# RolandFaure/metagenome_vector_sketches

Measured on AMD Instinct MI355X. Metric: samples projected/sec + pairwise Jaccard cells/sec, d=2048, 1/2/4/8 GPUs, higher is better.
Workload: dtype u64 hash -> int32 sketch; int8 limbs x int32 MFMA accumulate; fp64 keep test

## Files before the change

### metagenome_vector_sketches_amd/csrc/mvs_capi.hip

```cpp
#include "mvs_capi_internal.h"

using namespace mvs_capi;

namespace mvs {
int capi_fail(int code, const char* fmt, ...);
hipStream_t capi_stream(mvs_ctx* c) { return c->stream; }
int capi_device(mvs_ctx* c) { return c->device; }
const Options& capi_options(mvs_ctx* c) { return c->opt; }
}

namespace {
thread_local std::string g_err;
}

std::atomic<unsigned long long> mvs_capi::g_set_ids{0};

int mvs_capi::fail(int code, const char* fmt, ...) {
    char buf[512];
    va_list ap;
    va_start(ap, fmt);
    vsnprintf(buf, sizeof buf, fmt, ap);
    va_end(ap);
    g_err = buf;
    return code;
}

int mvs::capi_fail(int code, const char* fmt, ...) {
    char buf[512];
    va_list ap;
    va_start(ap, fmt);
    vsnprintf(buf, sizeof buf, fmt, ap);
    va_end(ap);
    g_err = buf;
    return code;
}

namespace {

struct Roctx {
    int (*push)(const char*) = nullptr;
    int (*pop)() = nullptr;
    Roctx() {
        for (const char* name : {"librocprofiler-sdk-roctx.so.1", "librocprofiler-sdk-roctx.so", "libroctx64.so.4",
                                 "libroctx64.so", "/opt/rocm/lib/librocprofiler-sdk-roctx.so"}) {
            if (void* h = dlopen(name, RTLD_NOW | RTLD_LOCAL)) {
                push = reinterpret_cast<int (*)(const char*)>(dlsym(h, "roctxRangePushA"));
                pop = reinterpret_cast<int (*)()>(dlsym(h, "roctxRangePop"));
                if (push && pop) return;
                push = nullptr;
                pop = nullptr;
            }
        }
    }
};
const Roctx& roctx() {
    static const Roctx r;
    return r;
}

}

namespace mvs_capi {

Range::Range(const mvs_ctx* c, const char* name) {
    if (c && c->opt.markers && roctx().push) {
        roctx().push(name);
        on = true;
    }
}
Range::~Range() {
    if (on) roctx().pop();
}

int ensure_buf(mvs_ctx* c, void** p, size_t* have, size_t bytes) {
    if (*have >= bytes) return MVS_OK;
    if (*p) {
        HIP_TRY(hipStreamSynchronize(c->stream));
        HIP_TRY(hipFree(*p));
        *p = nullptr;
        *have = 0;
    }
    const size_t want = bytes + std::min<size_t>(bytes / 4, (size_t)256 << 20) + 4096;
    if (hipMalloc(p, want) != hipSuccess) return fail(MVS_E_NOMEM, "hipMalloc of %zu bytes failed", want);
    *have = want;
    return MVS_OK;
}

int ensure_read_back(mvs_ctx* c, size_t total) {
    if (c->rb_pinned && c->rb_bytes >= total) return MVS_OK;
    if (c->rb_pinned) HIP_TRY(hipHostFree(c->rb_pinned));
    c->rb_pinned = nullptr;
    c->rb_bytes = 0;
    const size_t want = std::max<size_t>(total * 2, (size_t)1 << 20);
    HIP_TRY(hipHostMalloc(&c->rb_pinned, want, hipHostMallocDefault));
    c->rb_bytes = want;
    return MVS_OK;
}
int read_back(mvs_ctx* c, hipStream_t st, std::initializer_list<ReadBack> items) {
    size_t total = 0;
    for (const ReadBack& it : items) total += (it.bytes + 63) & ~(size_t)63;
    const int rc_rb = ensure_read_back(c, total);
    if (rc_rb) return rc_rb;
    size_t at = 0;
    for (const ReadBack& it : items) {
        if (it.bytes) HIP_TRY(hipMemcpyAsync((char*)c->rb_pinned + at, it.src, it.bytes, hipMemcpyDeviceToHost, st));
        at += (it.bytes + 63) & ~(size_t)63;
    }
    HIP_TRY(hipStreamSynchronize(st));
    at = 0;
    for (const ReadBack& it : items) {
        if (it.bytes) memcpy(it.dst, (const char*)c->rb_pinned + at, it.bytes);
        at += (it.bytes + 63) & ~(size_t)63;
    }
    return MVS_OK;
}

int ensure_scratch(mvs_ctx* c, size_t bytes) {
    if (c->scratch_bytes >= bytes) return MVS_OK;
    if (c->scratch) {
        HIP_TRY(hipStreamSynchronize(c->stream));
        HIP_TRY(hipFree(c->scratch));
        c->scratch = nullptr;
        c->scratch_bytes = 0;
    }
    HIP_TRY(hipMalloc(&c->scratch, bytes));
    c->scratch_bytes = bytes;
    return MVS_OK;
}

int acquire_pinned(mvs_ctx* c, size_t bytes) {
    if (c->pinned_busy) {
        HIP_TRY(hipEventSynchronize(c->pinned_ev));
        c->pinned_busy = false;
    }
    if (c->pinned_bytes >= bytes) return MVS_OK;
    if (c->pinned) {
        HIP_TRY(hipHostFree(c->pinned));
        c->pinned = nullptr;
        c->pinned_bytes = 0;
    }
    const size_t want = bytes < (1u << 20) ? (1u << 20) : bytes;
    HIP_TRY(hipHostMalloc(&c->pinned, want, hipHostMallocDefault));
    c->pinned_bytes = want;
    return MVS_OK;
}

struct OptionSpec {
    const char* name;
    int mvs::Options::*ifield;
    double mvs::Options::*dfield;
    long long lo, hi;
};
const OptionSpec kOptions[] = {
    {"pairwise_filter", &mvs::Options::pairwise_filter, nullptr, 0, 2},
    {"filter_variant", &mvs::Options::filter_variant, nullptr, -1, 99},
    {"exact_variant", &mvs::Options::exact_variant, nullptr, 0, 3},
    {"pairwise_variant", &mvs::Options::pairwise_variant, nullptr, 0, 9},
    {"pairwise_symmetric", &mvs::Options::pairwise_symmetric, nullptr, 0, 1},
    {"pairwise_debug", &mvs::Options::pairwise_debug, nullptr, 0, 15},
    {"sort", &mvs::Options::sort, nullptr, 0, 2},
    {"enable_k3", &mvs::Options::enable_k3, nullptr, 0, 1},
    {"markers", &mvs::Options::markers, nullptr, 0, 1},
    {"project_variant", &mvs::Options::project_variant, nullptr, 0, 14},
    {"comm_timeout_s", &mvs::Options::comm_timeout_s, nullptr, 1, 86400},
    {"pairwise_map", &mvs::Options::pairwise_map, nullptr, 0, 2},
    {"coarse_radix", &mvs::Options::coarse_radix, nullptr, 0, 1},
    {"cand_regions", &mvs::Options::cand_regions, nullptr, 0, 1},
    {"recheck_mode", &mvs::Options::recheck_mode, nullptr, 0, 3},
    {"recheck_blocks", &mvs::Options::recheck_blocks, nullptr, 1, 64},
    {"stream_dense", &mvs::Options::stream_dense, nullptr, 0, 5},
    {"encode_stage_words", &mvs::Options::encode_stage_words, nullptr, 1, 64},
    {"stream_block_rows", &mvs::Options::stream_block_rows, nullptr, 0, 1 << 30},
    {"tile_dense_thr", &mvs::Options::tile_dense_thr, nullptr, 0, 8192},
    {"stream_list_cells", &mvs::Options::stream_list_cells, nullptr, 0, 1 << 30},
    {"stream_pipeline", &mvs::Options::stream_pipeline, nullptr, 0, 1},
    {"stream_trace", &mvs::Options::stream_trace, nullptr, 0, 1},
    {"search_stream", &mvs::Options::search_stream, nullptr, 0, 1},
    {"search_depth", &mvs::Options::search_depth, nullptr, 3, 6},
    {"fragment_major", &mvs::Options::fragment_major, nullptr, 0, 1},
    {"pairwise_bdirect", &mvs::Options::pairwise_bdirect, nullptr, 0, 1},
    {"plan_strip_wgs", &mvs::Options::plan_strip_wgs, nullptr, 256, 1 << 22},
    {"recode_rows_wg", &mvs::Options::recode_rows_wg, nullptr, 8, 16},
    {"plan_speculate", &mvs::Options::plan_speculate, nullptr, 0, 1},
    {"plan_order", &mvs::Options::plan_order, nullptr, 0, 1},
    {"stream_piece_mib", &mvs::Options::stream_piece_mib, nullptr, 1, 1024},
    {"stream_spec", &mvs::Options::stream_spec, nullptr, 0, 1},
    {"stream_copy", &mvs::Options::stream_copy, nullptr, 0, 1},
    {"topk_dots", &mvs::Options::topk_dots, nullptr, 0, 1},
    {"topk_block_rows", &mvs::Options::topk_block_rows, nullptr, 0, 1 << 30},
    {"pairwise_block_cells", nullptr, &mvs::Options::pairwise_block_cells, 1, (1LL << 62)},
};

int apply_option(mvs::Options& o, const OptionSpec& sp, long long v) {
#ifndef MVS_ABLATIONS
    if (sp.ifield == &mvs::Options::pairwise_debug && v != 0)
        return fail(MVS_E_INVALID, "pairwise_debug needs a library built with -DMVS_ABLATIONS");
    if (sp.ifield == &mvs::Options::filter_variant && v >= 11 && v <= 33)
        return fail(MVS_E_INVALID, "filter_variant %lld is a k-loop ablation: needs -DMVS_ABLATIONS", v);
#endif
    if (v < sp.lo || v > sp.hi) return fail(MVS_E_INVALID, "option %s: %lld outside [%lld, %lld]", sp.name, v, sp.lo, sp.hi);
    if (sp.ifield) o.*(sp.ifield) = (int)v;
    else o.*(sp.dfield) = (double)v;
    return MVS_OK;
}

void options_from_env(mvs::Options& o) {
    for (const OptionSpec& sp : kOptions) {
        std::string env = "MVS_";
        for (const char* p = sp.name; *p; ++p) env += (char)toupper((unsigned char)*p);
        const char* e = getenv(env.c_str());
        if (!e || !*e) continue;
        long long v;
        if (sp.ifield == &mvs::Options::sort && (e[0] == 'm' || e[0] == 'r')) v = e[0] == 'r' ? 2 : 1;
        else v = sp.dfield ? (long long)atof(e) : atoll(e);
        const std::string keep = g_err;
        if (apply_option(o, sp, v) != MVS_OK) g_err = keep;
    }
}

void parallel_copy(void* dst, const void* src, size_t bytes) {
    const size_t kMin = 8u << 20;
    unsigned nt = std::thread::hardware_concurrency();
    nt = nt == 0 ? 4 : (nt > 16 ? 16 : nt);
    if (bytes < 2 * kMin) nt = 1;
    if (nt <= 1) {
        std::memcpy(dst, src, bytes);
        return;
    }
    std::vector<std::thread> pool;
    const size_t per = (bytes / nt + 4095) & ~(size_t)4095;
    for (unsigned t = 0; t < nt; ++t) {
        const size_t b = (size_t)t * per;
        if (b >= bytes) break;
        const size_t n = std::min(per, bytes - b);
        pool.emplace_back([=]() { std::memcpy((char*)dst + b, (const char*)src + b, n); });
    }
    for (auto& th : pool) th.join();
}

int ensure_upload_pipeline(mvs_ctx* c) {
    if (c->up_bytes) return MVS_OK;
    HIP_TRY(hipStreamCreateWithFlags(&c->up_stream, hipStreamNonBlocking));
    for (int i = 0; i < 2; ++i) {
        HIP_TRY(hipHostMalloc(&c->up_pinned[i], kUploadPiece, hipHostMallocDefault));
        HIP_TRY(hipEventCreateWithFlags(&c->up_done[i], hipEventDisableTiming));
    }
    c->up_bytes = kUploadPiece;
    return MVS_OK;
}

int check_kernel(const char* what) {
    hipError_t e = hipGetLastError();
    if (e != hipSuccess) return fail(MVS_E_HIP, "%s launch: %s", what, hipGetErrorString(e));
    return MVS_OK;
}

}

extern "C" {

const char* mvs_version(void) { return "mvs_hip 0.1 (gfx950)"; }
const char* mvs_last_error(void) { return g_err.c_str(); }

int mvs_device_count(int* count) {
    if (!count) return fail(MVS_E_INVALID, "count is NULL");
    int n = 0;
    hipError_t e = hipGetDeviceCount(&n);
    if (e != hipSuccess) {
        *count = 0;
        return fail(MVS_E_HIP, "hipGetDeviceCount: %s", hipGetErrorString(e));
    }
    *count = n;
    return MVS_OK;
}

int mvs_ctx_create(int device, mvs_ctx** out) {
    if (!out) return fail(MVS_E_INVALID, "ctx out pointer is NULL");
    *out = nullptr;
    int n = 0;
    hipError_t e = hipGetDeviceCount(&n);
    if (e != hipSuccess || n <= 0)
        return fail(MVS_E_HIP, "no HIP device available (%s); libmvs_hip has no CPU fallback",
                    e != hipSuccess ? hipGetErrorString(e) : "device count 0");
    if (device < 0 || device >= n) return fail(MVS_E_INVALID, "device %d out of range [0,%d)", device, n);
    HIP_TRY(hipSetDevice(device));
    hipDeviceProp_t prop;
    HIP_TRY(hipGetDeviceProperties(&prop, device));
    if (std::strncmp(prop.gcnArchName, "gfx950", 6) != 0)
        return fail(MVS_E_HIP, "device %d is %s; this library is built for gfx950 only", device, prop.gcnArchName);
    mvs_ctx* c = new (std::nothrow) mvs_ctx();
    if (!c) return fail(MVS_E_NOMEM, "out of host memory");
    c->device = device;
#ifdef MVS_ABLATIONS
    c->opt.pairwise_bdirect = 0;
#endif
    options_from_env(c->opt);
    if (hipStreamCreateWithFlags(&c->own_stream, hipStreamNonBlocking) != hipSuccess) {
        delete c;
        return fail(MVS_E_HIP, "hipStreamCreate failed");
    }
    c->stream = c->own_stream;
    for (auto& ev : c->ev) {
        if (hipEventCreate(&ev) != hipSuccess) {
            mvs_ctx_destroy(c);
            return fail(MVS_E_HIP, "hipEventCreate failed");
        }
    }
    if (hipEventCreateWithFlags(&c->pinned_ev, hipEventDisableTiming) != hipSuccess) {
        mvs_ctx_destroy(c);
        return fail(MVS_E_HIP, "hipEventCreate failed");
    }
    if (hipMalloc((void**)&c->d_counter, 2048) != hipSuccess) {
        mvs_ctx_destroy(c);
        return fail(MVS_E_HIP, "hipMalloc failed");
    }
    *out = c;
// ... 264 lines not shown
```

### metagenome_vector_sketches_amd/csrc/mvs_capi_sketch.hip

```cpp
#include "mvs_capi_internal.h"

using namespace mvs_capi;

extern "C" {

int mvs_project_csr(mvs_ctx* c, const uint64_t* hashes, int mem_hashes, const int64_t* offsets,
                    int64_t n_samples, int d, int32_t* out, int mem_out) {
    return mvs_project_csr_stats(c, hashes, mem_hashes, offsets, n_samples, d, out, mem_out, nullptr, nullptr);
}

int mvs_project_csr_stats(mvs_ctx* c, const uint64_t* hashes, int mem_hashes, const int64_t* offsets,
                          int64_t n_samples, int d, int32_t* out, int mem_out, int64_t* sumsq, int64_t* max_abs) {
    if (!c) return fail(MVS_E_INVALID, "ctx is NULL");
    const Range range(c, "mvs_project_csr");
    if ((sumsq == nullptr) != (max_abs == nullptr)) return fail(MVS_E_INVALID, "sumsq and max_abs go together");
    int64_t* const sumsq_user = sumsq;
    DevBuf dsum;
    if (max_abs) *max_abs = 0;
    if (n_samples < 0 || d <= 0) return fail(MVS_E_INVALID, "n_samples=%lld d=%d", (long long)n_samples, d);
    if (!mem_ok(mem_hashes) || !mem_ok(mem_out)) return fail(MVS_E_INVALID, "bad mem flag");
    if (n_samples == 0) return MVS_OK;
    if (!offsets || !out) return fail(MVS_E_INVALID, "offsets/out is NULL");
    HIP_TRY(hipSetDevice(c->device));

    if (n_samples >= (1LL << 31)) return fail(MVS_E_RANGE, "too many samples");
    size_t n_units = 0;
    bool all_single = true;
    for (int64_t s = 0; s < n_samples; ++s) {
        const int64_t b = offsets[s], e = offsets[s + 1];
        if (e < b) return fail(MVS_E_INVALID, "offsets not monotone at sample %lld", (long long)s);
        if (e - b >= (1LL << 31)) return fail(MVS_E_RANGE, "sample %lld has >= 2^31 hashes", (long long)s);
        n_units += e == b ? 1 : (size_t)((e - b + mvs::kProjUnitMax - 1) / mvs::kProjUnitMax);
        all_single = all_single && (e - b) <= mvs::kProjUnitMax;
    }
    int rc = acquire_pinned(c, std::max<size_t>(n_units * sizeof(mvs::ProjUnit), 256));
    if (rc) return rc;
    mvs::ProjUnit* units = (mvs::ProjUnit*)c->pinned;
    {
        size_t w = 0;
        for (int64_t s = 0; s < n_samples; ++s) {
            const int64_t b = offsets[s], e = offsets[s + 1];
            const bool single = (e - b) <= mvs::kProjUnitMax;
            if (e == b) units[w++] = mvs::ProjUnit{b, 0, (int32_t)s, 1, 0};
            for (int64_t p = b; p < e; p += mvs::kProjUnitMax) {
                mvs::ProjUnit u;
                u.begin = p;
                u.count = (int32_t)std::min<int64_t>(mvs::kProjUnitMax, e - p);
                u.sample = (int32_t)s;
                u.single = single ? 1 : 0;
                u.pad = 0;
                units[w++] = u;
            }
        }
    }
    const int64_t total = offsets[n_samples];
    if (total > 0 && !hashes) return fail(MVS_E_INVALID, "hashes is NULL");

    DevBuf dh, dout;
    const uint64_t* d_hashes = hashes;
    const bool pipelined = mem_hashes == MVS_MEM_HOST && (size_t)total * 8 > kUploadPiece;
    if (mem_hashes == MVS_MEM_HOST) {
        HIP_TRY(dh.alloc((size_t)total * 8));
        if (!pipelined) HIP_TRY(hipMemcpyAsync(dh.p, hashes, (size_t)total * 8, hipMemcpyHostToDevice, c->stream));
        d_hashes = (const uint64_t*)dh.p;
    }
    int32_t* d_out = out;
    const size_t out_bytes = (size_t)n_samples * (size_t)d * 4;
    if (mem_out == MVS_MEM_HOST) {
        HIP_TRY(dout.alloc(out_bytes));
        d_out = (int32_t*)dout.p;
        if (sumsq) {
            HIP_TRY(dsum.alloc((size_t)n_samples * 8));
            sumsq = (int64_t*)dsum.p;
        }
    }
    const size_t ubytes = n_units * sizeof(mvs::ProjUnit);
    rc = ensure_scratch(c, std::max<size_t>(ubytes, 256));
    if (rc) return rc;
    if (n_units) {
        HIP_TRY(hipMemcpyAsync(c->scratch, units, ubytes, hipMemcpyHostToDevice, c->stream));
        HIP_TRY(hipEventRecord(c->pinned_ev, c->stream));
        c->pinned_busy = true;
    }

    if (!all_single) HIP_TRY(hipMemsetAsync(d_out, 0, out_bytes, c->stream));
    const bool fused = sumsq != nullptr && all_single;
    if (fused) {
        HIP_TRY(hipMemsetAsync(sumsq, 0, (size_t)n_samples * 8, c->stream));
        HIP_TRY(hipMemsetAsync(c->d_counter, 0, 8, c->stream));
    }
    if (c->timing) HIP_TRY(hipEventRecord(c->ev[0], c->stream));
    const int nblk = (d + 63) / 64;
    int bpw = (nblk % 4 == 0 && nblk >= 8) ? 14 : (nblk >= 2 ? 2 : 1);
    if (c->opt.project_variant == 14 && nblk >= 4) bpw = 14;
    if (c->opt.project_variant == 12 && nblk >= 2) bpw = 12;
    if (c->opt.project_variant == 2 && nblk >= 2) bpw = 2;
    if (c->opt.project_variant == 1) bpw = 1;
    if (!pipelined) {
        mvs::launch_project(c->stream, d_hashes, (const mvs::ProjUnit*)c->scratch, (int64_t)n_units, d, d_out, bpw,
                            fused ? (unsigned long long*)sumsq : nullptr, fused ? c->d_counter : nullptr);
        rc = check_kernel("k_project");
        if (rc) return rc;
    } else {
        rc = ensure_upload_pipeline(c);
        if (rc) return rc;
        size_t u_done = 0;
        const size_t total_bytes = (size_t)total * 8;
        int piece = 0;
        for (size_t off = 0; off < total_bytes; off += kUploadPiece, ++piece) {
            const int b = piece & 1;
            const size_t len = std::min(kUploadPiece, total_bytes - off);
            if (piece >= 2) HIP_TRY(hipEventSynchronize(c->up_done[b]));
            parallel_copy(c->up_pinned[b], (const char*)hashes + off, len);
            HIP_TRY(hipMemcpyAsync((char*)dh.p + off, c->up_pinned[b], len, hipMemcpyHostToDevice, c->up_stream));
            HIP_TRY(hipEventRecord(c->up_done[b], c->up_stream));
            const int64_t covered = (int64_t)((off + len) / 8);
            size_t u_next = u_done;
            while (u_next < n_units && units[u_next].begin + units[u_next].count <= covered) ++u_next;
            if (u_next > u_done) {
                HIP_TRY(hipStreamWaitEvent(c->stream, c->up_done[b], 0));
                mvs::launch_project(c->stream, d_hashes, (const mvs::ProjUnit*)c->scratch + u_done, (int64_t)(u_next - u_done), d,
                                    d_out, bpw, fused ? (unsigned long long*)sumsq : nullptr, fused ? c->d_counter : nullptr);
                rc = check_kernel("k_project");
                if (rc) return rc;
                u_done = u_next;
            }
        }
        if (u_done != n_units) return fail(MVS_E_INVALID, "internal: %zu of %zu projection units launched", u_done, n_units);
    }
    if (c->timing) {
        HIP_TRY(hipEventRecord(c->ev[1], c->stream));
        c->ev_valid[0] = true;
    }
    if (sumsq) {
        if (fused) {
            unsigned long long m = 0;
            {
                const int rb_rc = read_back(c, c->stream, {{&m, c->d_counter, 8}});
                if (rb_rc) return rb_rc;
            }
            *max_abs = (int64_t)m;
        } else {
            rc = mvs_sketch_stats(c, d_out, MVS_MEM_DEVICE, n_samples, d, sumsq, MVS_MEM_DEVICE, max_abs);
            if (rc) return rc;
        }
    }
    if (mem_out == MVS_MEM_HOST) {
        HIP_TRY(hipMemcpyAsync(out, d_out, out_bytes, hipMemcpyDeviceToHost, c->stream));
        if (sumsq_user) HIP_TRY(hipMemcpyAsync(sumsq_user, sumsq, (size_t)n_samples * 8, hipMemcpyDeviceToHost, c->stream));
        HIP_TRY(hipStreamSynchronize(c->stream));
    } else if (mem_hashes == MVS_MEM_HOST) {
        HIP_TRY(hipStreamSynchronize(c->stream));
    } else {
    }
    return MVS_OK;
}

int mvs_sketch_sumsq(mvs_ctx* c, const int32_t* sketches, int mem_in, int64_t n, int d, int64_t* sumsq,
                     int mem_out) {
    if (!c) return fail(MVS_E_INVALID, "ctx is NULL");
    if (n < 0 || d <= 0 || !mem_ok(mem_in) || !mem_ok(mem_out)) return fail(MVS_E_INVALID, "bad argument");
    if (n == 0) return MVS_OK;
    if (!sketches || !sumsq) return fail(MVS_E_INVALID, "NULL buffer");
    HIP_TRY(hipSetDevice(c->device));
    DevBuf din, dout;
    const int32_t* d_in = sketches;
    if (mem_in == MVS_MEM_HOST) {
        HIP_TRY(din.alloc((size_t)n * d * 4));
        HIP_TRY(hipMemcpyAsync(din.p, sketches, (size_t)n * d * 4, hipMemcpyHostToDevice, c->stream));
        d_in = (const int32_t*)din.p;
    }
    int64_t* d_out = sumsq;
    if (mem_out == MVS_MEM_HOST) {
        HIP_TRY(dout.alloc((size_t)n * 8));
        d_out = (int64_t*)dout.p;
    }
    mvs::launch_sumsq(c->stream, d_in, n, d, d_out);
    int rc = check_kernel("k_sumsq");
    if (rc) return rc;
    if (mem_out == MVS_MEM_HOST)
        HIP_TRY(hipMemcpyAsync(sumsq, d_out, (size_t)n * 8, hipMemcpyDeviceToHost, c->stream));
    if (mem_out == MVS_MEM_HOST || mem_in == MVS_MEM_HOST) HIP_TRY(hipStreamSynchronize(c->stream));
    return MVS_OK;
}

}

namespace mvs_capi {

__device__ double norm_sq_from_text(long long sumsq, int d) {
    if (sumsq <= 0) return 0.0;
    const double x = sqrt((double)sumsq / (double)d);
    constexpr double p10[23] = {1e0,  1e1,  1e2,  1e3,  1e4,  1e5,  1e6,  1e7,  1e8,  1e9,  1e10, 1e11,
                                1e12, 1e13, 1e14, 1e15, 1e16, 1e17, 1e18, 1e19, 1e20, 1e21, 1e22};
    int e = 0;
    if (x >= 1.0) {
        while (e < 21 && x >= p10[e + 1]) ++e;
    } else {
        double y = x;
        while (e > -16 && y < 1.0) {
            y *= 10.0;
            --e;
        }
    }
    int j = 5 - e;
    double m, err;
    if (j >= 0) {
        m = x * p10[j];
        err = fma(x, p10[j], -m);
    } else {
        m = x / p10[-j];
        err = -fma(m, p10[-j], -x);
    }
    double r = rint(m);
    const double fl = floor(m);
    if (m - fl == 0.5 && err != 0.0) r = err > 0.0 ? fl + 1.0 : fl;
    if (r >= 1e6) {
        r = 1e5;
        --j;
    }
    const double v = j >= 0 ? r / p10[j] : r * p10[-j];
    return v * v;
}

__global__ __launch_bounds__(256) void k_norms_sq_text(const int64_t* __restrict__ sumsq, int64_t n, int d,
                                                       double* __restrict__ out) {
    const int64_t i = (int64_t)blockIdx.x * 256 + threadIdx.x;
    if (i < n) out[i] = norm_sq_from_text(sumsq[i], d);
}

}

extern "C" {

int mvs_norms_sq_text(mvs_ctx* c, const int64_t* sumsq, int64_t n, int d, double* out) {
    if (!c) return fail(MVS_E_INVALID, "ctx is NULL");
    if (n < 0 || d <= 0) return fail(MVS_E_INVALID, "bad argument");
    if (n == 0) return MVS_OK;
    if (!sumsq || !out) return fail(MVS_E_INVALID, "NULL buffer");
    if ((n + 255) / 256 > 0x7fffffffLL) return fail(MVS_E_INVALID, "too many entries");
    HIP_TRY(hipSetDevice(c->device));
    hipLaunchKernelGGL(k_norms_sq_text, dim3((unsigned)((n + 255) / 256)), dim3(256), 0, c->stream, sumsq, n, d, out);
    return check_kernel("k_norms_sq_text");
}

int mvs_sketch_stats(mvs_ctx* c, const int32_t* sketches, int mem_in, int64_t n, int d, int64_t* sumsq, int mem_out,
// ... 350 lines not shown
```

### metagenome_vector_sketches_amd/csrc/mvs_project.hip

```cpp
#include "mvs_internal.h"

namespace mvs {

namespace {

constexpr int kLV = 11;
constexpr uint64_t kGolden = 0x9e3779b97f4a7c15ULL;

__device__ __forceinline__ uint32_t xor3(uint32_t a, uint32_t b, uint32_t c) {
    return __builtin_amdgcn_bitop3_b32(a, b, c, 0x96);
}
__device__ __forceinline__ uint32_t maj3(uint32_t a, uint32_t b, uint32_t c) {
    return __builtin_amdgcn_bitop3_b32(a, b, c, 0xE8);
}

__device__ __forceinline__ uint64_t splitmix_tail(uint64_t z) {
    z = (z ^ (z >> 30)) * 0xbf58476d1ce4e5b9ULL;
    z = (z ^ (z >> 27)) * 0x94d049bb133111ebULL;
    return z ^ (z >> 31);
}

template <int BPW>
struct Acc {
    uint32_t lo[BPW][kLV];
    uint32_t hi[BPW][kLV];
};

template <int LEVEL, int BPW, class Gen>
__device__ __forceinline__ void absorb(Acc<BPW>& s, Gen& g, uint32_t (&clo)[BPW], uint32_t (&chi)[BPW]) {
    if constexpr (LEVEL == 0) {
        g.next(clo, chi);
    } else {
        uint32_t alo[BPW], ahi[BPW], blo[BPW], bhi[BPW];
        absorb<LEVEL - 1, BPW>(s, g, alo, ahi);
        absorb<LEVEL - 1, BPW>(s, g, blo, bhi);
#pragma unroll
        for (int b = 0; b < BPW; ++b) {
            const uint32_t tl = s.lo[b][LEVEL - 1], th = s.hi[b][LEVEL - 1];
            clo[b] = maj3(tl, alo[b], blo[b]);
            chi[b] = maj3(th, ahi[b], bhi[b]);
            s.lo[b][LEVEL - 1] = xor3(tl, alo[b], blo[b]);
            s.hi[b][LEVEL - 1] = xor3(th, ahi[b], bhi[b]);
        }
    }
}

template <int FROM, int BPW>
__device__ __forceinline__ void ripple(Acc<BPW>& s, uint32_t (&clo)[BPW], uint32_t (&chi)[BPW]) {
#pragma unroll
    for (int l = FROM; l < kLV; ++l) {
#pragma unroll
        for (int b = 0; b < BPW; ++b) {
            const uint32_t tl = s.lo[b][l] & clo[b], th = s.hi[b][l] & chi[b];
            s.lo[b][l] ^= clo[b];
            s.hi[b][l] ^= chi[b];
            clo[b] = tl;
            chi[b] = th;
        }
    }
}

template <int BPW, bool MASKED>
struct BatchGen {
    const uint64_t (&h)[8];
    const uint64_t (&cb)[BPW];
    int64_t remaining;
    int j = 0;
    __device__ __forceinline__ BatchGen(const uint64_t (&h_)[8], const uint64_t (&cb_)[BPW], int64_t rem)
        : h(h_), cb(cb_), remaining(rem) {}
    __device__ __forceinline__ void next(uint32_t (&lo)[BPW], uint32_t (&hi)[BPW]) {
        const uint64_t hv = h[j];
        bool valid = true;
        if constexpr (MASKED) valid = (int64_t)j * 64 < remaining;
        ++j;
#pragma unroll
        for (int b = 0; b < BPW; ++b) {
            uint64_t x = splitmix_tail(hv + cb[b]);
            if constexpr (MASKED) x = valid ? x : 0ULL;
            lo[b] = (uint32_t)x;
            hi[b] = (uint32_t)(x >> 32);
        }
    }
};

constexpr uint32_t kC1Lo = 0x1ce4e5b9u, kC1Hi = 0xbf58476du;

template <int BPW>
struct BatchGenShared {
    const uint64_t (&x)[8];
    int j = 0;
    __device__ __forceinline__ explicit BatchGenShared(const uint64_t (&x_)[8]) : x(x_) {}
    __device__ __forceinline__ void next(uint32_t (&lo)[BPW], uint32_t (&hi)[BPW]) {
        const uint64_t x0 = x[j++];
        const uint64_t t = x0 >> 30;
        const uint32_t x0l = (uint32_t)x0, tl = (uint32_t)t;
        const uint32_t zh = (uint32_t)(x0 >> 32) ^ (uint32_t)(t >> 32);
        const uint32_t p = zh * kC1Lo;
#pragma unroll
        for (int b = 0; b < BPW; ++b) {
            const uint32_t zl = (x0l + 64u * (uint32_t)b) ^ tl;
            const uint64_t m = (uint64_t)zl * (uint64_t)kC1Lo;
            const uint32_t whi = (uint32_t)(m >> 32) + zl * kC1Hi + p;
            uint64_t w = ((uint64_t)whi << 32) | (uint64_t)(uint32_t)m;
            w = (w ^ (w >> 27)) * 0x94d049bb133111ebULL;
            w ^= w >> 31;
            lo[b] = (uint32_t)w;
            hi[b] = (uint32_t)(w >> 32);
        }
    }
};

__device__ __forceinline__ bool hazard(const uint64_t (&h)[8], uint64_t cb0, uint64_t (&x)[8]) {
    uint32_t least = 0xffffffffu;
#pragma unroll
    for (int j = 0; j < 8; ++j) {
        x[j] = h[j] + cb0;
        const uint32_t xl = (uint32_t)x[j];
        const uint32_t miss = ~xl & 0x3fffff00u;
        least = miss < least ? miss : least;
    }
    return __any(least == 0u) != 0;
}

template <bool CLAMP>
__device__ __forceinline__ void load_batch(uint64_t (&h)[8], const uint64_t* base, int64_t pos, int lane,
                                           int64_t last) {
    if constexpr (CLAMP) {
#pragma unroll
        for (int j = 0; j < 8; ++j) {
            int64_t idx = pos + j * 64 + lane;
            idx = idx < last ? idx : last;
            h[j] = base[idx];
        }
    } else {
        const uint64_t* p = base + pos + lane;
#pragma unroll
        for (int j = 0; j < 8; ++j) h[j] = p[j * 64];
    }
}

template <int LV0>
__device__ __forceinline__ int32_t reduce_counts(const uint32_t (&lo_in)[kLV], const uint32_t (&hi_in)[kLV],
                                                 int lane) {
    static_assert(LV0 >= 1 && LV0 <= kLV, "live digits");
    constexpr int kOut = LV0 + 6;
    uint32_t lo[kOut], hi[kOut];
#pragma unroll
    for (int l = 0; l < kOut; ++l) {
        lo[l] = l < LV0 ? lo_in[l] : 0u;
        hi[l] = l < LV0 ? hi_in[l] : 0u;
    }
#pragma unroll
    for (int s = 0; s < 6; ++s) {
        uint32_t cl = 0, ch = 0;
#pragma unroll
        for (int l = 0; l < LV0 + s + 1; ++l) {
            const uint32_t pl = (uint32_t)__shfl_xor((int)lo[l], 1 << s, 64);
            const uint32_t ph = (uint32_t)__shfl_xor((int)hi[l], 1 << s, 64);
            const uint32_t sl = xor3(lo[l], pl, cl), sh = xor3(hi[l], ph, ch);
            cl = maj3(lo[l], pl, cl);
            ch = maj3(hi[l], ph, ch);
            lo[l] = sl;
            hi[l] = sh;
        }
    }
    int32_t cnt = 0;
    const int sh = lane & 31;
#pragma unroll
    for (int l = 0; l < kOut; ++l) {
        const uint32_t w = lane < 32 ? lo[l] : hi[l];
        cnt += (int32_t)((w >> sh) & 1u) << l;
    }
    return cnt;
}

template <int BPW, bool STATS, bool SHARED = false>
__global__ __launch_bounds__(256) void k_project(const uint64_t* __restrict__ hashes,
                                                 const ProjUnit* __restrict__ units, long long n_units, int ny,
                                                 int d, int nblk, int32_t* __restrict__ out,
                                                 unsigned long long* __restrict__ sumsq,
                                                 unsigned long long* __restrict__ max_abs) {
    const int lane = threadIdx.x & 63;
    const int wave = __builtin_amdgcn_readfirstlane(threadIdx.x >> 6);
    const long long grp = (long long)blockIdx.x / (8 * ny);
    const int rem = (int)((long long)blockIdx.x % (8 * ny));
    const long long unit = grp * 8 + (rem & 7);
    const int y = rem >> 3;
    if (unit >= n_units) return;
    const int b0 = (y * 4 + wave) * BPW;
    if (b0 >= nblk) return;
    const ProjUnit u = units[unit];
    const uint64_t* base = hashes + u.begin;
    const int64_t count = u.count;

    Acc<BPW> s;
#pragma unroll
    for (int b = 0; b < BPW; ++b)
#pragma unroll
        for (int l = 0; l < kLV; ++l) s.lo[b][l] = s.hi[b][l] = 0u;

    uint64_t cb[BPW];
#pragma unroll
    for (int b = 0; b < BPW; ++b) cb[b] = (uint64_t)(b0 + b) * 64ULL + kGolden;

    if (count > 0) {
        const int64_t last = count - 1;
        const int64_t nfull = count >> 9;
        uint64_t hv[8], hn[8];
        load_batch<true>(hv, base, 0, lane, last);
        int64_t b = 0;
        for (; b + 4 < nfull; b += 4) {
            uint32_t c8lo[4][BPW], c8hi[4][BPW];
#pragma unroll
            for (int sb = 0; sb < 4; ++sb) {
                load_batch<false>(hn, base, (b + sb + 1) << 9, lane, last);
                uint64_t xv[8];
                if (SHARED && !hazard(hv, cb[0], xv)) {
                    BatchGenShared<BPW> g(xv);
                    absorb<3, BPW>(s, g, c8lo[sb], c8hi[sb]);
                } else {
                    BatchGen<BPW, false> g(hv, cb, 0);
                    absorb<3, BPW>(s, g, c8lo[sb], c8hi[sb]);
                }
#pragma unroll
                for (int j = 0; j < 8; ++j) hv[j] = hn[j];
            }
            uint32_t c16lo[2][BPW], c16hi[2][BPW], c32lo[BPW], c32hi[BPW];
#pragma unroll
            for (int h2 = 0; h2 < 2; ++h2)
#pragma unroll
                for (int q = 0; q < BPW; ++q) {
                    const uint32_t tl = s.lo[q][3], th = s.hi[q][3];
                    c16lo[h2][q] = maj3(tl, c8lo[2 * h2][q], c8lo[2 * h2 + 1][q]);
                    c16hi[h2][q] = maj3(th, c8hi[2 * h2][q], c8hi[2 * h2 + 1][q]);
                    s.lo[q][3] = xor3(tl, c8lo[2 * h2][q], c8lo[2 * h2 + 1][q]);
                    s.hi[q][3] = xor3(th, c8hi[2 * h2][q], c8hi[2 * h2 + 1][q]);
                }
#pragma unroll
            for (int q = 0; q < BPW; ++q) {
                const uint32_t tl = s.lo[q][4], th = s.hi[q][4];
                c32lo[q] = maj3(tl, c16lo[0][q], c16lo[1][q]);
                c32hi[q] = maj3(th, c16hi[0][q], c16hi[1][q]);
                s.lo[q][4] = xor3(tl, c16lo[0][q], c16lo[1][q]);
                s.hi[q][4] = xor3(th, c16hi[0][q], c16hi[1][q]);
            }
            ripple<5, BPW>(s, c32lo, c32hi);
        }
        for (; b < nfull; ++b) {
            load_batch<true>(hn, base, (b + 1) << 9, lane, last);
            BatchGen<BPW, false> g(hv, cb, 0);
            uint32_t clo[BPW], chi[BPW];
            absorb<3, BPW>(s, g, clo, chi);
            ripple<3, BPW>(s, clo, chi);
#pragma unroll
            for (int j = 0; j < 8; ++j) hv[j] = hn[j];
        }
        if ((count & 511) != 0) {
            const int rem = (int)(count & 511);
            BatchGen<BPW, true> g(hv, cb, count - (nfull << 9) - lane);
            uint32_t clo[BPW], chi[BPW];
            if (rem <= 64) {
                absorb<0, BPW>(s, g, clo, chi);
                ripple<0, BPW>(s, clo, chi);
            } else if (rem <= 128) {
                absorb<1, BPW>(s, g, clo, chi);
                ripple<1, BPW>(s, clo, chi);
            } else if (rem <= 256) {
                absorb<2, BPW>(s, g, clo, chi);
                ripple<2, BPW>(s, clo, chi);
            } else {
                absorb<3, BPW>(s, g, clo, chi);
                ripple<3, BPW>(s, clo, chi);
            }
        }
    }

    long long ss = 0;
    unsigned int mx = 0;
#pragma unroll
    for (int b = 0; b < BPW; ++b) {
        if (b0 + b >= nblk) break;
        int32_t cnt;
        if (count <= 64) cnt = reduce_counts<1>(s.lo[b], s.hi[b], lane);
        else if (count <= 64 * 15) cnt = reduce_counts<4>(s.lo[b], s.hi[b], lane);
        else if (count <= 64 * 127) cnt = reduce_counts<7>(s.lo[b], s.hi[b], lane);
        else if (count <= 64 * 511) cnt = reduce_counts<9>(s.lo[b], s.hi[b], lane);
        else cnt = reduce_counts<kLV>(s.lo[b], s.hi[b], lane);
        const int k = (b0 + b) * 64 + lane;
        if (k < d) {
            const int32_t v = (int32_t)count - 2 * cnt;
            int32_t* dst = out + (int64_t)u.sample * d + k;
            if (u.single)
                *dst = v;
            else
                atomicAdd(dst, v);
            if (STATS) {
                ss += (long long)v * v;
                const unsigned int av = (unsigned int)(v < 0 ? -v : v);
                mx = av > mx ? av : mx;
            }
        }
    }
    if (STATS) {
#pragma unroll
        for (int o = 32; o > 0; o >>= 1) {
            ss += __shfl_xor(ss, o, 64);
            const unsigned int other = (unsigned int)__shfl_xor((int)mx, o, 64);
            mx = other > mx ? other : mx;
        }
        if (lane == 0) {
            atomicAdd(sumsq + u.sample, (unsigned long long)ss);
            if (mx > *reinterpret_cast<volatile unsigned long long*>(max_abs)) atomicMax(max_abs, (unsigned long long)mx);
        }
    }
}

__global__ __launch_bounds__(256) void k_sumsq(const int32_t* __restrict__ sk, int64_t n, int d,
                                               int64_t* __restrict__ out) {
    const int lane = threadIdx.x & 63;
    const int64_t row = (int64_t)blockIdx.x * 4 + (threadIdx.x >> 6);
    if (row >= n) return;
    const int32_t* p = sk + row * d;
    long long acc = 0;
    for (int k = lane; k < d; k += 64) {
        const long long v = p[k];
        acc += v * v;
    }
#pragma unroll
    for (int o = 32; o > 0; o >>= 1) acc += __shfl_xor(acc, o, 64);
    if (lane == 0) out[row] = acc;
}

__global__ __launch_bounds__(256) void k_stats(const int32_t* __restrict__ sk, int64_t n, int d,
                                               int64_t* __restrict__ sumsq, unsigned long long* __restrict__ max_abs) {
    const int lane = threadIdx.x & 63;
    const int64_t row = (int64_t)blockIdx.x * 4 + (threadIdx.x >> 6);
    if (row >= n) return;
    const int32_t* p = sk + row * d;
    long long acc = 0;
    unsigned int m = 0;
    if ((d & 3) == 0 && ((uintptr_t)p & 15) == 0) {
        const int4* p4 = reinterpret_cast<const int4*>(p);
        for (int k = lane; k < d / 4; k += 64) {
            const int4 v = p4[k];
            const long long a = v.x, b = v.y, c = v.z, e = v.w;
            acc += a * a + b * b + c * c + e * e;
            const unsigned int ma = (unsigned int)(a < 0 ? -a : a), mb = (unsigned int)(b < 0 ? -b : b);
            const unsigned int mc = (unsigned int)(c < 0 ? -c : c), me = (unsigned int)(e < 0 ? -e : e);
            m = max(max(m, max(ma, mb)), max(mc, me));
        }
    } else {
        for (int k = lane; k < d; k += 64) {
            const long long v = p[k];
            acc += v * v;
            m = max(m, (unsigned int)(v < 0 ? -v : v));
        }
    }
#pragma unroll
    for (int o = 32; o > 0; o >>= 1) {
        acc += __shfl_xor(acc, o, 64);
        m = max(m, (unsigned int)__shfl_xor((int)m, o, 64));
    }
    if (lane == 0) {
        sumsq[row] = acc;
        if (m > *reinterpret_cast<volatile unsigned long long*>(max_abs)) atomicMax(max_abs, (unsigned long long)m);
    }
}

__global__ __launch_bounds__(256) void k_saturate_i16(const int32_t* __restrict__ in, int64_t n,
                                                      int16_t* __restrict__ out) {
    const int64_t stride = (int64_t)gridDim.x * blockDim.x;
    for (int64_t i = (int64_t)blockIdx.x * blockDim.x + threadIdx.x; i < n; i += stride) {
        const int32_t v = in[i];
        out[i] = (int16_t)(v > 32767 ? 32767 : (v < -32768 ? -32768 : v));
    }
}

}

template <int BPW, bool SHARED>
static void launch_project_as(hipStream_t stream, unsigned grid, bool stats, const uint64_t* d_hashes, const ProjUnit* d_units,
                              long long nu, int ny, int d, int nblk, int32_t* d_out, unsigned long long* d_sumsq,
                              unsigned long long* d_max_abs) {
    if (stats)
        hipLaunchKernelGGL((k_project<BPW, true, SHARED>), dim3(grid), dim3(256), 0, stream, d_hashes, d_units, nu, ny, d, nblk,
                           d_out, d_sumsq, d_max_abs);
    else
        hipLaunchKernelGGL((k_project<BPW, false, SHARED>), dim3(grid), dim3(256), 0, stream, d_hashes, d_units, nu, ny, d, nblk,
                           d_out, d_sumsq, d_max_abs);
}

int launch_project(hipStream_t stream, const uint64_t* d_hashes, const ProjUnit* d_units, int64_t n_units,
                   int d, int32_t* d_out, int variant, unsigned long long* d_sumsq, unsigned long long* d_max_abs) {
    if (n_units == 0) return 0;
    const int nblk = (d + 63) / 64;
    const int bpw = variant % 10;
    const int ny = (nblk + 4 * bpw - 1) / (4 * bpw);
    const int64_t kMaxUnits = ((int64_t)(0xffffffffLL / 256) / (8 * ny) - 1) * 8;
    for (int64_t u0 = 0; u0 < n_units; u0 += kMaxUnits) {
        const int64_t nu = n_units - u0 < kMaxUnits ? n_units - u0 : kMaxUnits;
        const unsigned grid = (unsigned)(((nu + 7) / 8) * 8 * ny);
        const bool stats = d_sumsq != nullptr;
        switch (variant) {
            case 1: launch_project_as<1, false>(stream, grid, stats, d_hashes, d_units + u0, (long long)nu, ny, d, nblk, d_out, d_sumsq, d_max_abs); break;
            case 12: launch_project_as<2, true>(stream, grid, stats, d_hashes, d_units + u0, (long long)nu, ny, d, nblk, d_out, d_sumsq, d_max_abs); break;
            case 14: launch_project_as<4, true>(stream, grid, stats, d_hashes, d_units + u0, (long long)nu, ny, d, nblk, d_out, d_sumsq, d_max_abs); break;
            default: launch_project_as<2, false>(stream, grid, stats, d_hashes, d_units + u0, (long long)nu, ny, d, nblk, d_out, d_sumsq, d_max_abs); break;
        }
    }
    return 0;
}

constexpr int64_t kRowSlab = (int64_t)4 << 22;

int launch_sumsq(hipStream_t stream, const int32_t* d_sk, int64_t n, int d, int64_t* d_out) {
    for (int64_t r0 = 0; r0 < n; r0 += kRowSlab) {
        const int64_t m = n - r0 < kRowSlab ? n - r0 : kRowSlab;
        hipLaunchKernelGGL(k_sumsq, dim3((unsigned)((m + 3) / 4)), dim3(256), 0, stream, d_sk + r0 * d, m, d, d_out + r0);
    }
    return 0;
}

int launch_stats(hipStream_t stream, const int32_t* d_sk, int64_t n, int d, int64_t* d_sumsq,
                 unsigned long long* d_max_abs) {
    for (int64_t r0 = 0; r0 < n; r0 += kRowSlab) {
        const int64_t m = n - r0 < kRowSlab ? n - r0 : kRowSlab;
        hipLaunchKernelGGL(k_stats, dim3((unsigned)((m + 3) / 4)), dim3(256), 0, stream, d_sk + r0 * d, m, d, d_sumsq + r0,
                           d_max_abs);
    }
    return 0;
}

int launch_saturate_i16(hipStream_t stream, const int32_t* d_in, int64_t n, int16_t* d_out) {
    if (n == 0) return 0;
    int64_t blocks = (n + 255) / 256;
    if (blocks > 4096) blocks = 4096;
    hipLaunchKernelGGL(k_saturate_i16, dim3((unsigned)blocks), dim3(256), 0, stream, d_in, n, d_out);
    return 0;
}

}
```

Measured before the change: 1.058 million.

## Add deep carry-save projection variant with DPP/permlane wave reductions as default

```diff
diff --git a/metagenome_vector_sketches_amd/csrc/mvs_capi.hip b/metagenome_vector_sketches_amd/csrc/mvs_capi.hip
--- a/metagenome_vector_sketches_amd/csrc/mvs_capi.hip
+++ b/metagenome_vector_sketches_amd/csrc/mvs_capi.hip
@@ -161,7 +161,7 @@
     {"sort", &mvs::Options::sort, nullptr, 0, 2},
     {"enable_k3", &mvs::Options::enable_k3, nullptr, 0, 1},
     {"markers", &mvs::Options::markers, nullptr, 0, 1},
-    {"project_variant", &mvs::Options::project_variant, nullptr, 0, 14},
+    {"project_variant", &mvs::Options::project_variant, nullptr, 0, 24},
     {"comm_timeout_s", &mvs::Options::comm_timeout_s, nullptr, 1, 86400},
     {"pairwise_map", &mvs::Options::pairwise_map, nullptr, 0, 2},
     {"coarse_radix", &mvs::Options::coarse_radix, nullptr, 0, 1},
diff --git a/metagenome_vector_sketches_amd/csrc/mvs_capi_sketch.hip b/metagenome_vector_sketches_amd/csrc/mvs_capi_sketch.hip
--- a/metagenome_vector_sketches_amd/csrc/mvs_capi_sketch.hip
+++ b/metagenome_vector_sketches_amd/csrc/mvs_capi_sketch.hip
@@ -91,7 +91,8 @@
     }
     if (c->timing) HIP_TRY(hipEventRecord(c->ev[0], c->stream));
     const int nblk = (d + 63) / 64;
-    int bpw = (nblk % 4 == 0 && nblk >= 8) ? 14 : (nblk >= 2 ? 2 : 1);
+    int bpw = (nblk % 4 == 0 && nblk >= 8) ? 24 : (nblk >= 2 ? 2 : 1);
+    if (c->opt.project_variant == 24 && nblk >= 4) bpw = 24;
     if (c->opt.project_variant == 14 && nblk >= 4) bpw = 14;
     if (c->opt.project_variant == 12 && nblk >= 2) bpw = 12;
     if (c->opt.project_variant == 2 && nblk >= 2) bpw = 2;
diff --git a/metagenome_vector_sketches_amd/csrc/mvs_project.hip b/metagenome_vector_sketches_amd/csrc/mvs_project.hip
--- a/metagenome_vector_sketches_amd/csrc/mvs_project.hip
+++ b/metagenome_vector_sketches_amd/csrc/mvs_project.hip
@@ -174,7 +174,87 @@
     return cnt;
 }
 
-template <int BPW, bool STATS, bool SHARED = false>
+__device__ __forceinline__ void add_digit(uint32_t& w, uint32_t a, uint32_t b, uint32_t& c) {
+    w = xor3(a, b, c);
+    c = maj3(a, b, c);
+}
+
+template <int CTRL>
+__device__ __forceinline__ uint32_t dpp_mov(uint32_t x) {
+    return (uint32_t)__builtin_amdgcn_update_dpp(0, (int)x, CTRL, 0xf, 0xf, false);
+}
+
+template <int CTRL, int LIVE, int N>
+__device__ __forceinline__ void reduce_stage_dpp(uint32_t (&w)[N]) {
+    static_assert(LIVE < N, "room for the carry");
+    uint32_t c = 0;
+#pragma unroll
+    for (int l = 0; l < LIVE; ++l) {
+        add_digit(w[l], w[l], dpp_mov<CTRL>(w[l]), c);
+    }
+    w[LIVE] = c;
+}
+
+template <int LV0>
+__device__ __forceinline__ int32_t reduce_counts_valu(const uint32_t (&lo_in)[kLV], const uint32_t (&hi_in)[kLV],
+                                                      int lane) {
+    static_assert(LV0 >= 1 && LV0 <= kLV, "live digits");
+    constexpr int kOut = LV0 + 6;
+    uint32_t w[kOut];
+    uint32_t c = 0;
+#pragma unroll
+    for (int l = 0; l < LV0; ++l) {
+        const auto r = __builtin_amdgcn_permlane32_swap(lo_in[l], hi_in[l], false, false);
+        add_digit(w[l], r[0], r[1], c);
+    }
+    w[LV0] = c;
+#pragma unroll
+    for (int l = LV0 + 1; l < kOut; ++l) w[l] = 0u;
+    reduce_stage_dpp<0xb1, LV0 + 1>(w);
+    reduce_stage_dpp<0x4e, LV0 + 2>(w);
+    reduce_stage_dpp<0x141, LV0 + 3>(w);
+    reduce_stage_dpp<0x140, LV0 + 4>(w);
+    c = 0;
+#pragma unroll
+    for (int l = 0; l < LV0 + 5; ++l) {
+        const auto r = __builtin_amdgcn_permlane16_swap(w[l], w[l], false, false);
+        add_digit(w[l], r[0], r[1], c);
+    }
+    w[LV0 + 5] = c;
+    int32_t cnt = 0;
+    const int sh = lane & 31;
+#pragma unroll
+    for (int l = 0; l < kOut; ++l) cnt += (int32_t)((w[l] >> sh) & 1u) << l;
+    return cnt;
+}
+
+template <int CTRL>
+__device__ __forceinline__ void sum_max_stage_dpp(unsigned long long& ss, uint32_t& mx) {
+    ss += ((unsigned long long)dpp_mov<CTRL>((uint32_t)(ss >> 32)) << 32) | dpp_mov<CTRL>((uint32_t)ss);
+    const uint32_t o = dpp_mov<CTRL>(mx);
+    mx = o > mx ? o : mx;
+}
+
+template <bool SWAP32>
+__device__ __forceinline__ void sum_max_stage_swap(unsigned long long& ss, uint32_t& mx) {
+    const uint32_t l = (uint32_t)ss, h = (uint32_t)(ss >> 32);
+    const auto rl = SWAP32 ? __builtin_amdgcn_permlane32_swap(l, l, false, false) : __builtin_amdgcn_permlane16_swap(l, l, false, false);
+    const auto rh = SWAP32 ? __builtin_amdgcn_permlane32_swap(h, h, false, false) : __builtin_amdgcn_permlane16_swap(h, h, false, false);
+    const auto rm = SWAP32 ? __builtin_amdgcn_permlane32_swap(mx, mx, false, false) : __builtin_amdgcn_permlane16_swap(mx, mx, false, false);
+    ss = (((unsigned long long)rh[0] << 32) | rl[0]) + (((unsigned long long)rh[1] << 32) | rl[1]);
+    mx = rm[0] > rm[1] ? rm[0] : rm[1];
+}
+
+__device__ __forceinline__ void wave_sum_max_valu(unsigned long long& ss, uint32_t& mx) {
+    sum_max_stage_dpp<0xb1>(ss, mx);
+    sum_max_stage_dpp<0x4e>(ss, mx);
+    sum_max_stage_dpp<0x141>(ss, mx);
+    sum_max_stage_dpp<0x140>(ss, mx);
+    sum_max_stage_swap<false>(ss, mx);
+    sum_max_stage_swap<true>(ss, mx);
+}
+
+template <int BPW, bool STATS, bool SHARED = false, bool DEEP = false>
 __global__ __launch_bounds__(256) void k_project(const uint64_t* __restrict__ hashes,
                                                  const ProjUnit* __restrict__ units, long long n_units, int ny,
                                                  int d, int nblk, int32_t* __restrict__ out,
@@ -209,6 +289,8 @@
         uint64_t hv[8], hn[8];
         load_batch<true>(hv, base, 0, lane, last);
         int64_t b = 0;
+        uint32_t p32lo[BPW], p32hi[BPW], p64lo[BPW], p64hi[BPW];
+        int grp4 = 0;
         for (; b + 4 < nfull; b += 4) {
             uint32_t c8lo[4][BPW], c8hi[4][BPW];
 #pragma unroll
@@ -244,7 +326,44 @@
                 s.lo[q][4] = xor3(tl, c16lo[0][q], c16lo[1][q]);
                 s.hi[q][4] = xor3(th, c16hi[0][q], c16hi[1][q]);
             }
-            ripple<5, BPW>(s, c32lo, c32hi);
+            if constexpr (DEEP) {
+                if (grp4 & 1) {
+                    uint32_t c64lo[BPW], c64hi[BPW];
+#pragma unroll
+                    for (int q = 0; q < BPW; ++q) {
+                        const uint32_t tl = s.lo[q][5], th = s.hi[q][5];
+                        c64lo[q] = maj3(tl, p32lo[q], c32lo[q]);
+                        c64hi[q] = maj3(th, p32hi[q], c32hi[q]);
+                        s.lo[q][5] = xor3(tl, p32lo[q], c32lo[q]);
+                        s.hi[q][5] = xor3(th, p32hi[q], c32hi[q]);
+                    }
+                    if (grp4 & 2) {
+                        uint32_t c128lo[BPW], c128hi[BPW];
+#pragma unroll
+                        for (int q = 0; q < BPW; ++q) {
+                            const uint32_t tl = s.lo[q][6], th = s.hi[q][6];
+                            c128lo[q] = maj3(tl, p64lo[q], c64lo[q]);
+                            c128hi[q] = maj3(th, p64hi[q], c64hi[q]);
+                            s.lo[q][6] = xor3(tl, p64lo[q], c64lo[q]);
+                            s.hi[q][6] = xor3(th, p64hi[q], c64hi[q]);
+                        }
+                        ripple<7, BPW>(s, c128lo, c128hi);
+                    } else {
+#pragma unroll
+                        for (int q = 0; q < BPW; ++q) p64lo[q] = c64lo[q], p64hi[q] = c64hi[q];
+                    }
+                } else {
+#pragma unroll
+                    for (int q = 0; q < BPW; ++q) p32lo[q] = c32lo[q], p32hi[q] = c32hi[q];
+                }
+                ++grp4;
+            } else {
+                ripple<5, BPW>(s, c32lo, c32hi);
+            }
+        }
+        if constexpr (DEEP) {
+            if (grp4 & 1) ripple<5, BPW>(s, p32lo, p32hi);
+            if (grp4 & 2) ripple<6, BPW>(s, p64lo, p64hi);
         }
         for (; b < nfull; ++b) {
             load_batch<true>(hn, base, (b + 1) << 9, lane, last);
@@ -281,7 +400,14 @@
     for (int b = 0; b < BPW; ++b) {
         if (b0 + b >= nblk) break;
         int32_t cnt;
-        if (count <= 64) cnt = reduce_counts<1>(s.lo[b], s.hi[b], lane);
+        if constexpr (DEEP) {
+            if (count <= 64) cnt = reduce_counts_valu<1>(s.lo[b], s.hi[b], lane);
+            else if (count <= 64 * 15) cnt = reduce_counts_valu<4>(s.lo[b], s.hi[b], lane);
+            else if (count <= 64 * 127) cnt = reduce_counts_valu<7>(s.lo[b], s.hi[b], lane);
+            else if (count <= 64 * 511) cnt = reduce_counts_valu<9>(s.lo[b], s.hi[b], lane);
+            else if (count <= 64 * 1023) cnt = reduce_counts_valu<10>(s.lo[b], s.hi[b], lane);
+            else cnt = reduce_counts_valu<kLV>(s.lo[b], s.hi[b], lane);
+        } else if (count <= 64) cnt = reduce_counts<1>(s.lo[b], s.hi[b], lane);
         else if (count <= 64 * 15) cnt = reduce_counts<4>(s.lo[b], s.hi[b], lane);
         else if (count <= 64 * 127) cnt = reduce_counts<7>(s.lo[b], s.hi[b], lane);
         else if (count <= 64 * 511) cnt = reduce_counts<9>(s.lo[b], s.hi[b], lane);
@@ -302,11 +428,19 @@
         }
     }
     if (STATS) {
-#pragma unroll
-        for (int o = 32; o > 0; o >>= 1) {
-            ss += __shfl_xor(ss, o, 64);
-            const unsigned int other = (unsigned int)__shfl_xor((int)mx, o, 64);
-            mx = other > mx ? other : mx;
+        if constexpr (DEEP) {
+            unsigned long long uss = (unsigned long long)ss;
+            uint32_t umx = mx;
+            wave_sum_max_valu(uss, umx);
+            ss = (long long)uss;
+            mx = umx;
+        } else {
+#pragma unroll
+            for (int o = 32; o > 0; o >>= 1) {
+                ss += __shfl_xor(ss, o, 64);
+                const unsigned int other = (unsigned int)__shfl_xor((int)mx, o, 64);
+                mx = other > mx ? other : mx;
+            }
         }
         if (lane == 0) {
             atomicAdd(sumsq + u.sample, (unsigned long long)ss);
@@ -378,15 +512,15 @@
 
 }
 
-template <int BPW, bool SHARED>
+template <int BPW, bool SHARED, bool DEEP = false>
 static void launch_project_as(hipStream_t stream, unsigned grid, bool stats, const uint64_t* d_hashes, const ProjUnit* d_units,
                               long long nu, int ny, int d, int nblk, int32_t* d_out, unsigned long long* d_sumsq,
                               unsigned long long* d_max_abs) {
     if (stats)
-        hipLaunchKernelGGL((k_project<BPW, true, SHARED>), dim3(grid), dim3(256), 0, stream, d_hashes, d_units, nu, ny, d, nblk,
+        hipLaunchKernelGGL((k_project<BPW, true, SHARED, DEEP>), dim3(grid), dim3(256), 0, stream, d_hashes, d_units, nu, ny, d, nblk,
                            d_out, d_sumsq, d_max_abs);
     else
-        hipLaunchKernelGGL((k_project<BPW, false, SHARED>), dim3(grid), dim3(256), 0, stream, d_hashes, d_units, nu, ny, d, nblk,
+        hipLaunchKernelGGL((k_project<BPW, false, SHARED, DEEP>), dim3(grid), dim3(256), 0, stream, d_hashes, d_units, nu, ny, d, nblk,
                            d_out, d_sumsq, d_max_abs);
 }
 
@@ -404,6 +538,7 @@
         switch (variant) {
             case 1: launch_project_as<1, false>(stream, grid, stats, d_hashes, d_units + u0, (long long)nu, ny, d, nblk, d_out, d_sumsq, d_max_abs); break;
             case 12: launch_project_as<2, true>(stream, grid, stats, d_hashes, d_units + u0, (long long)nu, ny, d, nblk, d_out, d_sumsq, d_max_abs); break;
+            case 24: launch_project_as<4, true, true>(stream, grid, stats, d_hashes, d_units + u0, (long long)nu, ny, d, nblk, d_out, d_sumsq, d_max_abs); break;
             case 14: launch_project_as<4, true>(stream, grid, stats, d_hashes, d_units + u0, (long long)nu, ny, d, nblk, d_out, d_sumsq, d_max_abs); break;
             default: launch_project_as<2, false>(stream, grid, stats, d_hashes, d_units + u0, (long long)nu, ny, d, nblk, d_out, d_sumsq, d_max_abs); break;
         }
```

New measurement: 1.091 million (median of 6 runs). 1.03x the previous value.
